# ooowedyn/InkLayer

Measured on AMD Instinct MI355X. Metric: sketches/sec end-to-end (GroundingDINO+SAM) at 1024x1024, higher is better.
Workload: dtype f16 (MFMA, f32 accumulate; f32 residual/norm/softmax; split-f16 = fp32-grade operands for patch-embed, neck, mask decoder); 1 GPU; full GroundingDINO Swin-T + SAM ViT-H pipeline, batch=8 per GPU, 1024x1024 synthetic sketches, 16 boxes/sketch, random-init weights; global_batch=8, parallelism=image-parallel x1

## Files before the change

### include/inklayer_hip.h

```cpp
#ifndef INKLAYER_HIP_H
#define INKLAYER_HIP_H

#include <stdint.h>

#ifdef __cplusplus
extern "C" {
#endif

#define INK_ABI_VERSION 8
int ink_abi_version(void);

typedef struct InkGemm {
  const void* A;
  const void* W;
  const float* bias;
  const float* col_scale;
  const float* residual;
  const int32_t* row_map;
  void* C;
  int32_t M, N, K;
  int32_t lda, ldw, ldr, ldc;
  int32_t act;
  int32_t c_f16;
} InkGemm;
#define INK_ACT_NONE 0
#define INK_ACT_GELU 1
#define INK_ACT_RELU 2
int ink_gemm_f16(const InkGemm* p, void* stream);
int ink_gemm_set_variant(int32_t v);
int ink_gemm_query_variant(int32_t M, int32_t N, int32_t K);

int ink_layernorm_rows(const float* x, int64_t ldx, const float* gamma, const float* beta,
                       float eps, const int32_t* gather, int32_t rows_out, int32_t C,
                       void* out_f16, float* out_f32, int64_t ldo, int32_t act, int32_t split,
                       const float* add, int64_t ld_add, const int32_t* add_batch_rows, int32_t rows_per_batch,
                       void* stream);

int ink_add_cvt_f16(const float* a, const float* b, int64_t n_b, void* out_f16, int64_t n,
                    void* stream);
int ink_add_split_f16(const float* a, const float* b, int64_t n_b, void* out_f16, int64_t n, int32_t C,
                      void* stream);
int ink_add_f32(const float* a, const float* b, int64_t n_b, float* out, int64_t n, void* stream);

typedef struct InkAttn {
  const void* Q; const void* K; const void* V;
  void* O;
  int64_t ldq, ldk, ldv, ldo;
  int32_t n_batch, n_heads, n_q, n_k, head_dim;
  float scale;
  int32_t bias_mode;
  int32_t grid_w;
  const int32_t* q_batch_rows;
  const int32_t* kv_batch_rows;
  const float* rel_h; const float* rel_w;
  const void* rel_aug;
  const float* dense_bias; const float* dense_mask;
  int32_t n_mask; int32_t rel_f16;
  const int32_t* tok_rows;
  const void* pad_k; const void* pad_v;
} InkAttn;
int ink_flash_attn(const InkAttn* p, void* stream);

int ink_relpos_bias64_f16(const void* Q, int64_t ldq, const float* rel_pos_h, const float* rel_pos_w, int32_t n_batch,
                          int32_t n_heads, int32_t head_dim, float scale, void* out_h_f16, void* out_w_f16, void* stream);

int ink_relpos_bias(const void* Q, int64_t ldq, const float* rel_pos_h, const float* rel_pos_w,
                    int32_t S, int32_t n_batch, int32_t n_heads, int32_t head_dim, float scale,
                    const int32_t* tok_rows, float* out_h, float* out_w, void* out_aug_f16,
                    void* stream);

int ink_sam_patchify(const void* image_u8, int32_t h, int32_t w, int32_t L, int32_t P,
                     const float* mean3, const float* std3, int32_t chan_reverse, int32_t split,
                     void* out_f16, void* stream);

int ink_resize_bilinear_u8(const void* src_u8, int32_t h, int32_t w, void* dst_u8, int32_t oh, int32_t ow,
                           const int32_t* xbounds, const int32_t* xcoef, int32_t kx,
                           const int32_t* ybounds, const int32_t* ycoef, int32_t ky, void* tmp_u8,
                           void* stream);

int ink_im2col3x3_f16(const void* in_f16, int32_t B, int32_t H, int32_t W, int32_t C, void* out_f16,
                      void* stream);

int ink_sam_pe_encode(const float* coords01, const float* gauss, int32_t N, int32_t F,
                      const float* add, int32_t n_add, float* out, void* stream);

int ink_sam_prompt_tokens(const float* points, const int32_t* labels, int32_t n_pts, int32_t pad, const float* boxes,
                          const float* gauss, int32_t F, const float* point_emb, const float* not_a_point,
                          const float* out_tok, float input_size, int32_t P, float* out, void* stream);

int ink_sam_mask_embed(const float* mask, const float* emb, const int32_t* emb_rows, const float* params,
                       int32_t n_params, float eps, int32_t P, int32_t g, float* keys, void* split_f16, void* stream);

int ink_sam_mask_logits(const float* up, const float* hyper, int32_t n, int32_t g, int32_t C,
                        float* out, void* stream);

int ink_sam_postprocess(const float* low, int32_t n, int32_t S, int32_t L, int32_t in_h,
                        int32_t in_w, int32_t out_h, int32_t out_w, float thr, void* out_u8,
                        float* out_logits, void* stream);

int ink_ms_deform_attn_forward(const float* value, const int64_t* spatial_shapes_host,
                               const int64_t* level_start_index_host, const float* sampling_loc,
                               const float* attn_weight, int32_t B, int32_t S, int32_t M, int32_t C,
                               int32_t Q, int32_t L, int32_t P, int32_t im2col_step, float* out,
                               void* stream);

int ink_ms_deform_attn_forward_dev(const void* value, const int64_t* spatial_shapes,
                                   const int64_t* level_start_index, const void* sampling_loc,
                                   const void* attn_weight, int32_t dtype, int32_t B, int32_t S, int32_t M,
                                   int32_t C, int32_t Q, int32_t L, int32_t P, int32_t im2col_step,
                                   void* out, void* stream);
int ink_ms_deform_attn_backward_dev(const void* value, const int64_t* spatial_shapes,
                                    const int64_t* level_start_index, const void* sampling_loc,
                                    const void* attn_weight, const void* grad_output, int32_t dtype,
                                    int32_t B, int32_t S, int32_t M, int32_t C, int32_t Q, int32_t L,
                                    int32_t P, int32_t im2col_step, void* grad_value,
                                    void* grad_sampling_loc, void* grad_attn_weight, void* stream);

int ink_msda_fused(const void* value_f16, const float* proj, int64_t ldp, const float* ref,
                   int32_t ref_dim, int64_t ref_q_stride, int64_t ref_b_stride,
                   const int32_t* shapes_host, int32_t B, int32_t S, int32_t Q, void* out_f16,
                   void* stream);

int ink_swin_patchify(const void* image_u8, int32_t h, int32_t w, const float* mean3,
                      const float* std3, void* out_f16, void* stream);

int ink_layernorm_merge4(const float* x, int64_t ldx, const float* gamma, const float* beta, float eps,
                         const int32_t* gather4, int32_t rows, int32_t C, void* out_f16, void* stream);

int ink_groupnorm_nhwc(const float* x, int32_t B, int32_t T, int32_t C, int32_t G, const float* gamma,
                       const float* beta, float eps, float* stats_ws, float* out,
                       int64_t out_batch_stride, void* stream);

int ink_gather_rows(const float* x, int64_t ldx, int64_t x_batch_rows, const int32_t* idx,
                    int64_t idx_batch_stride, int32_t rows_per_batch, int32_t B, int32_t C,
                    void* out_f16, float* out_f32, void* stream);

int ink_biattn_fusion(const void* QV_f16, const void* KL_f16, int32_t B, int32_t S, int32_t T, int32_t E,
                      float scale, float* scores_ws, float* stats_ws, float* partial_ws, int32_t chunk,
                      void* out_v_f16, void* out_l_f16, void* stream);

int ink_attn_fewkeys(const void* Q, int64_t ldq, const void* K, int64_t ldk, const void* V, int64_t ldv,
                     int32_t B, int32_t n_q, int32_t n_k, int32_t n_heads, int32_t head_dim, float scale,
                     const uint8_t* blocked, const int32_t* q_batch_rows, const float* q_add, int32_t io_f32, void* O,
                     int64_t ldo, void* stream);

int ink_attn_fewq(const void* Q, int64_t ldq, const void* K, int64_t ldk, const void* V, int64_t ldv,
                  int32_t n_batch, int32_t n_q, int32_t n_k, int32_t n_heads, int32_t head_dim, float scale,
                  const int32_t* q_batch_rows, const int32_t* kv_batch_rows, const float* k_add, void* O, int64_t ldo,
                  void* stream);

int ink_biattn_colstats(const float* scores, int32_t B, int32_t S, int32_t HT, float* part_ws, float* stats, void* stream);

int ink_fusion_fold_workspace(int32_t B, int32_t S, int64_t* out_floats);
int ink_fusion_fold(float* v_f32, int32_t B, int32_t S, const float* lnv_g, const float* lnv_b, float eps,
                    const float* text_k_f32, const float* text_vl_f32, int64_t ld_text, int32_t T, const void* Wq_f16,
                    const float* bq, const void* Wvv_f16, const float* bvv, const void* Wo_f16, const float* bo,
                    const float* gamma_v, float scale, float* ws, void* out_l_f16, const float* pos, void* out16_pos,
                    void* out16, void* stream);

int ink_sam_upscale_pack(const void* ws_f16, void* blob_f16, void* stream);
int ink_sam_upscale_tail(const float* u0, int64_t ld_tok, int32_t n, int32_t g, const float* ln_g, const float* ln_b, float eps,
                         const void* blob_f16, const float* b3, const float* hyper, int32_t n_masks, float* low,
                         void* stream);

int ink_proj256_ln_pack(const void* ws_f16, void* blob_f16, void* stream);
int ink_proj256_ln(const float* a_f32, const void* blob_f16, const float* bias, const float* res_f32,
                   const int32_t* res_batch_rows, int32_t rows_per_batch, const float* ln_g, const float* ln_b, float eps,
                   int64_t rows, float* out_f32, void* out_split_f16, void* stream);

int ink_ffn256_pack_bytes(int32_t hid, int32_t with_pre, int64_t* out_bytes);
int ink_ffn256_pack(const void* w1_f16, const float* b1, const void* w2_f16, int32_t hid, const void* wpre_f16, void* blob,
                    void* stream);
int ink_ffn256_fused(const void* x_f16, int64_t ldx, const float* res_f32, const void* blob, const float* b2,
                     const float* ln_g, const float* ln_b, float eps, int32_t M, int32_t hid, const float* pre_bias,
                     const float* pre_ln_g, const float* pre_ln_b, float* out_f32, void* stream);

int ink_topk_rowmax(const float* logits, int32_t B, int32_t S, int32_t T, int32_t K, int32_t* out_idx,
                    float* out_val, void* cand_ws, void* stream);

int ink_sine_embed4(const float* ref, const float* dim_t, int32_t N, void* out_f16, void* stream);

int ink_box_refine(const float* delta, int64_t ldd, const float* ref, int32_t N, int32_t ref_is_logit,
                   float* out, void* stream);
// ... 157 lines not shown
```

### inklayer_amd/_lib.py

```python
from __future__ import annotations

import ctypes as C
import os
from pathlib import Path

_LIB_PATH = Path(__file__).resolve().parent / "lib" / "libinklayer_hip.so"
_lib = None

c_void_p, c_int, c_i64, c_float = C.c_void_p, C.c_int32, C.c_int64, C.c_float


class InkGemm(C.Structure):
    _fields_ = [
        ("A", c_void_p), ("W", c_void_p), ("bias", c_void_p), ("col_scale", c_void_p),
        ("residual", c_void_p), ("row_map", c_void_p), ("C", c_void_p),
        ("M", c_int), ("N", c_int), ("K", c_int),
        ("lda", c_int), ("ldw", c_int), ("ldr", c_int), ("ldc", c_int),
        ("act", c_int), ("c_f16", c_int),
    ]


class InkAttn(C.Structure):
    _fields_ = [
        ("Q", c_void_p), ("K", c_void_p), ("V", c_void_p), ("O", c_void_p),
        ("ldq", c_i64), ("ldk", c_i64), ("ldv", c_i64), ("ldo", c_i64),
        ("n_batch", c_int), ("n_heads", c_int), ("n_q", c_int), ("n_k", c_int),
        ("head_dim", c_int), ("scale", c_float), ("bias_mode", c_int), ("grid_w", c_int),
        ("q_batch_rows", c_void_p), ("kv_batch_rows", c_void_p),
        ("rel_h", c_void_p), ("rel_w", c_void_p), ("rel_aug", c_void_p),
        ("dense_bias", c_void_p), ("dense_mask", c_void_p), ("n_mask", c_int), ("rel_f16", c_int),
        ("tok_rows", c_void_p), ("pad_k", c_void_p), ("pad_v", c_void_p),
    ]


SIGNATURES = {
    "ink_abi_version": [],
    "ink_gemm_f16": [C.POINTER(InkGemm), c_void_p],
    "ink_gemm_set_variant": [c_int],
    "ink_gemm_query_variant": [c_int, c_int, c_int],
    "ink_layernorm_rows": [c_void_p, c_i64, c_void_p, c_void_p, c_float, c_void_p, c_int, c_int,
                           c_void_p, c_void_p, c_i64, c_int, c_int, c_void_p, c_i64, c_void_p, c_int, c_void_p],
    "ink_add_split_f16": [c_void_p, c_void_p, c_i64, c_void_p, c_i64, c_int, c_void_p],
    "ink_add_cvt_f16": [c_void_p, c_void_p, c_i64, c_void_p, c_i64, c_void_p],
    "ink_add_f32": [c_void_p, c_void_p, c_i64, c_void_p, c_i64, c_void_p],
    "ink_flash_attn": [C.POINTER(InkAttn), c_void_p],
    "ink_sam_patchify": [c_void_p, c_int, c_int, c_int, c_int, C.POINTER(c_float), C.POINTER(c_float),
                         c_int, c_int, c_void_p, c_void_p],
    "ink_im2col3x3_f16": [c_void_p, c_int, c_int, c_int, c_int, c_void_p, c_void_p],
    "ink_resize_bilinear_u8": [c_void_p, c_int, c_int, c_void_p, c_int, c_int, c_void_p, c_void_p, c_int,
                               c_void_p, c_void_p, c_int, c_void_p, c_void_p],
    "ink_sam_pe_encode": [c_void_p, c_void_p, c_int, c_int, c_void_p, c_int, c_void_p, c_void_p],
    "ink_sam_mask_logits": [c_void_p, c_void_p, c_int, c_int, c_int, c_void_p, c_void_p],
    "ink_sam_prompt_tokens": [c_void_p, c_void_p, c_int, c_int, c_void_p, c_void_p, c_int, c_void_p, c_void_p,
                              c_void_p, c_float, c_int, c_void_p, c_void_p],
    "ink_sam_mask_embed": [c_void_p, c_void_p, c_void_p, c_void_p, c_int, c_float, c_int, c_int, c_void_p, c_void_p,
                           c_void_p],
    "ink_sam_postprocess": [c_void_p, c_int, c_int, c_int, c_int, c_int, c_int, c_int, c_float,
                            c_void_p, c_void_p, c_void_p],
    "ink_sam_amg_stats": [c_void_p, c_int, c_void_p, c_int, c_void_p, c_int, c_int, c_int, c_int, c_int, c_int, C.c_double,
                          C.c_double, c_int, c_int, c_int, c_int, c_void_p, c_void_p, c_void_p, c_void_p],
    "ink_mask_rle_counts": [c_void_p, c_void_p, c_int, c_int, c_int, c_void_p, c_void_p],
    "ink_mask_rle_write": [c_void_p, c_void_p, c_int, c_int, c_int, c_void_p, c_void_p, c_void_p],
    "ink_mask_small_regions_workspace_ints": [c_int, c_int, c_int, C.POINTER(c_i64)],
    "ink_mask_small_regions": [c_void_p, c_int, c_int, c_int, c_int, c_int, c_void_p, c_void_p, c_void_p, c_void_p,
                               c_void_p],
    "ink_box_nms": [c_void_p, c_void_p, c_int, c_float, c_void_p, c_void_p, c_void_p, c_void_p],
    "ink_ms_deform_attn_forward": [c_void_p, C.POINTER(c_i64), C.POINTER(c_i64), c_void_p, c_void_p, c_int,
                                   c_int, c_int, c_int, c_int, c_int, c_int, c_int, c_void_p, c_void_p],
    "ink_ms_deform_attn_forward_dev": [c_void_p, c_void_p, c_void_p, c_void_p, c_void_p, c_int, c_int, c_int, c_int,
                                       c_int, c_int, c_int, c_int, c_int, c_void_p, c_void_p],
    "ink_ms_deform_attn_backward_dev": [c_void_p, c_void_p, c_void_p, c_void_p, c_void_p, c_void_p, c_int, c_int, c_int,
                                        c_int, c_int, c_int, c_int, c_int, c_int, c_void_p, c_void_p, c_void_p,
                                        c_void_p],
    "ink_msda_fused": [c_void_p, c_void_p, c_i64, c_void_p, c_int, c_i64, c_i64, C.POINTER(c_int), c_int,
                       c_int, c_int, c_void_p, c_void_p],
    "ink_swin_patchify": [c_void_p, c_int, c_int, C.POINTER(c_float), C.POINTER(c_float), c_void_p, c_void_p],
    "ink_layernorm_merge4": [c_void_p, c_i64, c_void_p, c_void_p, c_float, c_void_p, c_int, c_int, c_void_p,
                             c_void_p],
    "ink_groupnorm_nhwc": [c_void_p, c_int, c_int, c_int, c_int, c_void_p, c_void_p, c_float, c_void_p,
                           c_void_p, c_i64, c_void_p],
    "ink_gather_rows": [c_void_p, c_i64, c_i64, c_void_p, c_i64, c_int, c_int, c_int, c_void_p, c_void_p,
                        c_void_p],
    "ink_biattn_fusion": [c_void_p, c_void_p, c_int, c_int, c_int, c_int, c_float, c_void_p, c_void_p,
                          c_void_p, c_int, c_void_p, c_void_p, c_void_p],
    "ink_biattn_colstats": [c_void_p, c_int, c_int, c_int, c_void_p, c_void_p, c_void_p],
    "ink_fusion_fold_workspace": [c_int, c_int, C.POINTER(c_i64)],
    "ink_relpos_bias64_f16": [c_void_p, c_i64, c_void_p, c_void_p, c_int, c_int, c_int, c_float, c_void_p, c_void_p, c_void_p],
    "ink_proj256_ln_pack": [c_void_p, c_void_p, c_void_p],
    "ink_proj256_ln": [c_void_p, c_void_p, c_void_p, c_void_p, c_void_p, c_int, c_void_p, c_void_p, c_float, c_i64, c_void_p,
                       c_void_p, c_void_p],
    "ink_sam_upscale_pack": [c_void_p, c_void_p, c_void_p],
    "ink_sam_upscale_tail": [c_void_p, c_i64, c_int, c_int, c_void_p, c_void_p, c_float, c_void_p, c_void_p, c_void_p,
                             c_int, c_void_p, c_void_p],
    "ink_ffn256_pack_bytes": [c_int, c_int, C.POINTER(c_i64)],
    "ink_ffn256_pack": [c_void_p, c_void_p, c_void_p, c_int, c_void_p, c_void_p, c_void_p],
    "ink_ffn256_fused": [c_void_p, c_i64, c_void_p, c_void_p, c_void_p, c_void_p, c_void_p, c_float, c_int, c_int,
                         c_void_p, c_void_p, c_void_p, c_void_p, c_void_p],
    "ink_fusion_fold": [c_void_p, c_int, c_int, c_void_p, c_void_p, c_float, c_void_p, c_void_p, c_i64, c_int, c_void_p,
                        c_void_p, c_void_p, c_void_p, c_void_p, c_void_p, c_void_p, c_float, c_void_p, c_void_p, c_void_p,
                        c_void_p, c_void_p, c_void_p],
    "ink_attn_fewkeys": [c_void_p, c_i64, c_void_p, c_i64, c_void_p, c_i64, c_int, c_int, c_int, c_int, c_int,
                         c_float, c_void_p, c_void_p, c_void_p, c_int, c_void_p, c_i64, c_void_p],
    "ink_attn_fewq": [c_void_p, c_i64, c_void_p, c_i64, c_void_p, c_i64, c_int, c_int, c_int, c_int, c_int,
                      c_float, c_void_p, c_void_p, c_void_p, c_void_p, c_i64, c_void_p],
    "ink_topk_rowmax": [c_void_p, c_int, c_int, c_int, c_int, c_void_p, c_void_p, c_void_p, c_void_p],
    "ink_sine_embed4": [c_void_p, c_void_p, c_int, c_void_p, c_void_p],
    "ink_box_refine": [c_void_p, c_i64, c_void_p, c_int, c_int, c_void_p, c_void_p],
    "ink_mask_cleanup_workspace_ints": [c_int, c_int, c_int, c_int, C.POINTER(c_i64)],
    "ink_mask_cleanup": [c_void_p, c_int, c_int, c_int, c_int, c_int, C.c_double, c_void_p, c_void_p, c_void_p,
                         c_void_p, c_void_p],
    "ink_mask_sketch_iou_counts": [c_void_p, c_void_p, c_int, c_int, c_int, c_void_p, c_void_p, c_void_p],
    "ink_refine_sketch_planes": [c_void_p, c_int, c_int, c_void_p, c_void_p, c_void_p],
    "ink_bitplane_pack": [c_void_p, c_int, c_int, c_int, c_int, c_void_p, c_void_p],
    "ink_refine_depth_samples": [c_void_p, c_int, c_void_p, c_void_p, c_int, c_int, c_int, c_void_p, c_void_p, c_void_p],
    "ink_refine_pair_tables": [c_void_p, c_void_p, c_int, c_int, c_int, c_void_p, c_void_p, c_void_p, c_void_p,
                               c_void_p, c_void_p],
    "ink_refine_composite": [c_void_p, c_void_p, c_int, c_int, c_int, c_void_p, c_void_p, c_void_p],
    "ink_refine_relabel_clean": [c_void_p, c_void_p, c_int, c_int, c_void_p, c_void_p],
    "ink_refine_grow_workspace": [c_int, c_int, C.POINTER(c_i64), C.POINTER(c_i64)],
    "ink_refine_grow": [c_void_p, c_void_p, c_int, c_int, c_void_p, c_void_p, c_void_p, c_void_p, c_void_p, c_void_p,
                        c_int, c_void_p, c_void_p],
    "ink_refine_query_dists": [c_void_p, c_void_p, c_void_p, c_int, c_int, c_int, c_void_p, c_void_p],
    "ink_refine_finalize": [c_void_p, c_void_p, c_int, c_void_p, c_int, c_int, c_void_p, c_void_p, c_void_p, c_void_p],
    "ink_host_sparse_sample": [c_void_p, c_int, c_int, c_void_p, c_int, c_void_p],
    "ink_host_assign_unlabeled": [c_void_p, c_int, c_void_p, c_int, c_void_p, c_void_p, c_void_p, c_int, c_void_p],
    "ink_depth_patchify": [c_void_p, c_int, c_int, c_int, c_int, c_int, c_int, C.POINTER(C.c_double), C.POINTER(C.c_double),
                           c_int, c_void_p, c_void_p],
    "ink_resize_bilinear_ac_nhwc": [c_void_p, c_int, c_int, c_int, c_int, c_int, c_int, c_void_p, c_void_p, c_void_p],
    "ink_im2col3x3_ex_f16": [c_void_p, c_int, c_int, c_int, c_int, c_int, c_int, c_void_p, c_void_p],
    "ink_conv3x3_f16": [c_void_p, c_int, c_int, c_int, c_int, c_void_p, c_int, c_void_p, c_int, c_int, c_int, c_void_p,
                        c_void_p, c_int, c_void_p],
    "ink_layers_otsu_planes": [c_void_p, c_int, c_int, c_int, c_int, c_void_p, c_void_p, c_void_p, c_void_p],
    "ink_layers_dilate": [c_void_p, c_int, c_int, c_int, c_int, c_int, c_void_p, c_void_p, c_void_p],
    "ink_layers_border_band": [c_void_p, c_int, c_int, c_int, c_int, c_void_p, c_void_p],
    "ink_layers_components_workspace_ints": [c_int, c_int, c_int, C.POINTER(c_i64)],
    "ink_layers_components": [c_void_p, c_int, c_int, c_int, c_int, c_void_p, c_void_p, c_void_p, c_void_p],
    "ink_layers_chamfer_workspace_ints": [c_int, c_int, c_int, C.POINTER(c_i64)],
    "ink_layers_chamfer": [c_void_p, c_void_p, c_int, c_int, c_int, c_int, c_int, c_void_p, c_void_p, c_void_p, c_void_p,
                           c_void_p, c_void_p],
    "ink_layers_mask_tables": [c_void_p, c_int, c_int, c_int, c_void_p, c_void_p, c_void_p],
    "ink_layers_assemble": [c_void_p, c_void_p, c_void_p, c_void_p, c_void_p, c_int, c_int, c_int, c_void_p, c_void_p,
                            c_void_p, c_void_p],
    "ink_layers_composite": [c_void_p, c_void_p, c_int, c_int, c_void_p, c_void_p],
    "ink_layers_gray": [c_void_p, c_int, c_int, c_int, c_void_p, c_void_p],
    "ink_layers_rgba": [c_void_p, c_void_p, c_int, c_int, c_int, c_void_p, c_void_p],
    "ink_inp_contrast": [c_void_p, c_int, c_int, c_float, c_void_p, c_void_p, c_void_p],
    "ink_inp_bilateral": [c_void_p, c_int, c_int, c_void_p, c_void_p, c_void_p],
    "ink_inp_mask_prepare": [c_void_p, c_int, c_int, c_int, c_int, c_void_p, c_void_p, c_void_p],
    "ink_inp_resize_u8": [c_void_p, c_int, c_int, c_int, c_void_p, c_int, c_int, c_void_p, c_void_p, c_int,
                          c_void_p, c_void_p, c_int, c_void_p, c_void_p],
    "ink_inp_condition": [c_void_p, c_void_p, c_int, c_int, c_void_p, c_void_p],
    "ink_inp_cleanup": [c_void_p, c_int, c_int, c_void_p, c_void_p, c_void_p, c_void_p, c_void_p],
    "ink_inp_soft_blend": [c_void_p, c_void_p, c_void_p, c_int, c_int, c_void_p, c_void_p, c_void_p, c_void_p],
    "ink_inp_luma": [c_void_p, c_int, c_int, c_int, c_void_p, c_void_p],
    "ink_inp_unsharp": [c_void_p, c_int, c_int, c_int, C.c_uint32, C.c_uint32, c_int, c_int, c_void_p, c_void_p, c_void_p],
    "ink_inp_rgba_cut": [c_void_p, c_void_p, c_int, c_int, c_void_p, c_void_p],
    "ink_vis_gray_min": [c_void_p, c_int, c_int, c_int, c_void_p, c_void_p],
    "ink_vis_colour": [c_void_p, c_int, c_void_p, c_int, c_int, c_void_p, c_void_p, c_int, c_int, c_void_p, c_void_p],
    "ink_eval_label_ranks": [c_void_p, c_int, c_int, c_int, c_void_p, c_void_p, c_int, c_void_p, c_void_p, c_void_p],
    "ink_eval_contingency": [c_void_p, c_int, c_int, c_void_p, c_int, c_void_p, c_int, c_int, c_int, c_int, c_void_p,
                             c_void_p],
    "ink_eval_label_boxes": [c_void_p, c_int, c_int, c_int, c_void_p, c_void_p],
    "ink_eval_paint_labels": [c_void_p, c_void_p, c_int, c_int, c_int, c_void_p, c_void_p],
    "ink_relpos_bias": [c_void_p, c_i64, c_void_p, c_void_p, c_int, c_int, c_int, c_int, c_float,
                        c_void_p, c_void_p, c_void_p, c_void_p, c_void_p],
}


class InkLayerHipError(RuntimeError):
    pass


def lib_path() -> Path:
    return Path(os.environ.get("INKLAYER_HIP_LIB", _LIB_PATH))


def lib() -> C.CDLL:
    global _lib
    if _lib is None:
        p = lib_path()
        if not p.exists():
            raise InkLayerHipError(
                f"{p} not found: build it with `python -m inklayer_amd.build` "
                "(there is no CPU/eager fallback for the InkLayer hot path)")
        try:
            import torch
        except ImportError:
            pass
        l = C.CDLL(str(p))
        for name, argtypes in SIGNATURES.items():
# ... 11 lines not shown
```

### inklayer_amd/csrc/gemm.hip

```cpp
#include <stdlib.h>

#include "common.h"
#include "../../include/inklayer_hip.h"

namespace {

template <int BK> struct Swz;
template <> struct Swz<64> {
  static __device__ __forceinline__ int f(int row) { return row & 7; }
};
template <> struct Swz<32> {
  static __device__ __forceinline__ int f(int row) { return (-(row >> 2)) & 3; }
};

typedef __attribute__((address_space(1))) const void* gptr_t;
typedef __attribute__((address_space(3))) void* lptr_t;

__device__ __forceinline__ bool residual_preloaded(const InkGemm& p) {
  return p.residual && p.act == INK_ACT_NONE && !p.col_scale;
}

template <int TM>
__device__ __forceinline__ void wave_rows(int (&rows)[TM], const InkGemm& p, int mw, int lane) {
#pragma unroll
  for (int ti = 0; ti < TM; ++ti) {
    const int m = mw + ti * 16 + (lane & 15);
    int r = -1;
    if (m < p.M) r = p.row_map ? p.row_map[m] : m;
    rows[ti] = r;
  }
}

template <int TM, int TN>
__device__ __forceinline__ void init_wave_tile(f32x4 (&acc)[TM][TN], const InkGemm& p, const int (&rows)[TM], int nw,
                                               int lane) {
  const int fq = lane >> 4;
  const bool pre = residual_preloaded(p);
#pragma unroll
  for (int ti = 0; ti < TM; ++ti) {
    const int r = pre ? rows[ti] : -1;
    const float* rp = p.residual + (size_t)max(r, 0) * p.ldr + nw + fq * 4;
#pragma unroll
    for (int j = 0; j < TN; ++j) {
      acc[ti][j] = (f32x4){0.f, 0.f, 0.f, 0.f};
      if (r >= 0 && nw + j * 16 + fq * 4 < p.N) acc[ti][j] = *(const f32x4*)(rp + j * 16);
    }
  }
}

template <int TM, int TN>
__device__ __forceinline__ void add_bias_wave_tile(f32x4 (&acc)[TM][TN], const InkGemm& p, int nw, int lane) {
  const int fq = lane >> 4;
#pragma unroll
  for (int j = 0; j < TN; ++j) {
    const int n = nw + j * 16 + fq * 4;
    f32x4 bv = (f32x4){0.f, 0.f, 0.f, 0.f};
    if (p.bias && n < p.N) bv = *(const f32x4*)(p.bias + n);
#pragma unroll
    for (int ti = 0; ti < TM; ++ti) acc[ti][j] += bv;
  }
}

template <int TM, int TN, int OUT, int MODE = -1>
__device__ __forceinline__ void store_wave_tile(f32x4 (&acc)[TM][TN], const InkGemm& p, char* er,
                                                const int (&rows)[TM], int nw, int lane) {
  constexpr bool F16O = OUT == 1;
  constexpr int WNC = TN * 16, EP = WNC * 4 + 16;
  constexpr int ES = OUT == 0 ? 4 : 8;
  constexpr int CPRW = WNC / ES;
  constexpr int NIT = (16 * CPRW + 63) / 64;
  const int fr = lane & 15, fq = lane >> 4;
  const bool wide16 = OUT != 0 && (p.ldc % 8 == 0);
  const bool res_late = MODE < 0 && p.residual && !residual_preloaded(p);
  const int act = MODE < 0 ? p.act : MODE;
  const bool scaled = MODE < 0 && p.col_scale != nullptr;
  int row_of[NIT], n_of[NIT];
#pragma unroll
  for (int it = 0; it < NIT; ++it) {
    const int c = it * 64 + lane;
    row_of[it] = c < 16 * CPRW ? c / CPRW : 16;
    n_of[it] = nw + (c % CPRW) * ES;
  }

  add_bias_wave_tile<TM, TN>(acc, p, nw, lane);

#pragma unroll
  for (int ti = 0; ti < TM; ++ti) {
#pragma unroll
    for (int j = 0; j < TN; ++j) {
      f32x4 v = acc[ti][j];
      if (act == INK_ACT_GELU) {
#pragma unroll
        for (int r = 0; r < 4; ++r) v[r] = gelu_erf(v[r]);
      } else if (act == INK_ACT_RELU) {
#pragma unroll
        for (int r = 0; r < 4; ++r) v[r] = fmaxf(v[r], 0.f);
      }
      if (scaled) {
        const int n = nw + j * 16 + fq * 4;
        if (n < p.N) v *= *(const f32x4*)(p.col_scale + n);
      }
      if (F16O) {
        *(f16x4*)(er + fr * EP + (j * 16 + fq * 4) * 2) = (f16x4){(f16)v[0], (f16)v[1], (f16)v[2], (f16)v[3]};
      } else {
        *(f32x4*)(er + fr * EP + (j * 16 + fq * 4) * 4) = v;
      }
    }
#pragma unroll
    for (int it = 0; it < NIT; ++it) {
      int r = __builtin_amdgcn_ds_bpermute((row_of[it] & 15) << 2, rows[ti]);
      if (row_of[it] >= 16 || n_of[it] >= p.N) r = -1;
      if (r >= 0) {
        const int c_n = n_of[it];
        const char* src = er + row_of[it] * EP + (c_n - nw) * (F16O ? 2 : 4);
        if (F16O) {
          f16x8 d = *(const f16x8*)src;
          f16* dst = (f16*)p.C + (size_t)r * p.ldc + c_n;
          if (res_late) {
            const float* rp = p.residual + (size_t)r * p.ldr + c_n;
#pragma unroll
            for (int e = 0; e < 8; ++e)
              if (c_n + e < p.N) d[e] = (f16)((float)d[e] + rp[e]);
          }
          if (wide16 && c_n + 8 <= p.N) {
            *(f16x8*)dst = d;
          } else {
            *(f16x4*)dst = (f16x4){d[0], d[1], d[2], d[3]};
            if (c_n + 8 <= p.N) *(f16x4*)(dst + 4) = (f16x4){d[4], d[5], d[6], d[7]};
          }
        } else {
          f32x4 d = *(const f32x4*)src;
          if (res_late) d += *(const f32x4*)(p.residual + (size_t)r * p.ldr + c_n);
          *(f32x4*)((float*)p.C + (size_t)r * p.ldc + c_n) = d;
        }
      }
    }
  }
}

__device__ __forceinline__ void tile_of(int id, int ntm, int ntn, int group_m, int& mt, int& nt) {
  if (group_m > 1) {
    const int per = group_m * ntn;
    const int first = (id / per) * group_m;
    const int gsz = min(ntm - first, group_m);
    mt = first + (id % per) % gsz;
    nt = (id % per) / gsz;
  } else {
    mt = id / ntn;
    nt = id % ntn;
  }
}

constexpr int NS = 2;
// ... 118 lines not shown
  constexpr int TM = 8, WNC = 16 * TN;
  constexpr int AHEAD = RING - 2;
  constexpr int AG = 4;
  constexpr int EP = WNC * 4 + 16;
  static_assert(8 * 16 * EP <= RING * GRAN, "patch fits");
  extern __shared__ __attribute__((aligned(16))) char smem[];
  const int tid = threadIdx.x, lane = tid & 63;
  const int wave = __builtin_amdgcn_readfirstlane(tid >> 6);
  const int grp = wave >> 2, wn = wave & 3;
  const int fr = lane & 15, fq = lane >> 4;

  const int ntn = (p.N + BN - 1) / BN, ntm = (p.M + BM - 1) / BM;
  int mt, nt;
  tile_of(xcd_remap(blockIdx.x, ntm * ntn), ntm, ntn, group_m, mt, nt);
  const int m0 = mt * BM, n0 = nt * BN;
  const int G = p.K / BK;
  const f16* __restrict__ A = (const f16*)p.A;
  const f16* __restrict__ W = (const f16*)p.W;
  const f16* srcA[IT_A];
  const f16* srcW[IT_W + (W_TAIL ? 1 : 0)];
#pragma unroll
  for (int it = 0; it < IT_A; ++it) {
    const int pch = it * NT + tid, row = pch / CPR, lch = (pch % CPR) ^ Swz<BK>::f(row);
    srcA[it] = A + (size_t)min(m0 + row, p.M - 1) * p.lda + lch * 8;
  }
#pragma unroll
  for (int it = 0; it < IT_W + (W_TAIL ? 1 : 0); ++it) {
    const int pch = it * NT + tid, row = min(pch / CPR, BN - 1), lch = (pch % CPR) ^ Swz<BK>::f(row);
    srcW[it] = W + (size_t)min(n0 + row, p.N - 1) * p.ldw + lch * 8;
  }
  auto dma = [&](int g, int slot) {
    char* base = smem + slot * GRAN;
#pragma unroll
    for (int it = 0; it < IT_A; ++it)
      __builtin_amdgcn_global_load_lds((gptr_t)(srcA[it] + g * BK), (lptr_t)(base + (it * NT + wave * 64) * 16), 16, 0, 0);
#pragma unroll
    for (int it = 0; it < IT_W; ++it)
      __builtin_amdgcn_global_load_lds((gptr_t)(srcW[it] + g * BK), (lptr_t)(base + TILE_A + (it * NT + wave * 64) * 16), 16, 0, 0);
    if (W_TAIL && grp == 0)
      __builtin_amdgcn_global_load_lds((gptr_t)(srcW[IT_W] + g * BK), (lptr_t)(base + TILE_A + (IT_W * NT + wave * 64) * 16), 16, 0, 0);
  };
  auto wait_ahead = [&]() {
    if (W_TAIL && grp == 0) {
      asm volatile("s_waitcnt vmcnt(%0)" ::"n"((AHEAD - 1) * (LOADS + 1)) : "memory");
    } else {
      asm volatile("s_waitcnt vmcnt(%0)" ::"n"((AHEAD - 1) * LOADS) : "memory");
    }
  };
  auto slot_end = [&]() {
    __builtin_amdgcn_sched_barrier(0);
    __builtin_amdgcn_s_barrier();
    __builtin_amdgcn_sched_barrier(0);
  };

  int rows[TM];
  wave_rows<TM>(rows, p, m0 + grp * 128, lane);
#pragma unroll
  for (int g = 0; g < AHEAD; ++g) dma(g, g);
  f32x4 acc[TM][TN];
  init_wave_tile<TM, TN>(acc, p, rows, n0 + wn * WNC, lane);
  if (residual_preloaded(p)) {
    asm volatile("s_waitcnt vmcnt(0)" ::: "memory");
  } else {
    wait_ahead();
  }
  slot_end();
  if (grp == 1) slot_end();

  const int offA = (grp * 128 + fr) * ROWB;
  const int offW = (wn * WNC + fr) * ROWB;
  const int co = (fq ^ Swz<BK>::f(fr)) << 4;
  f16x8 a[AG], w[TN];
  int cslot = 0, islot = AHEAD % RING;
  auto iter = [&](int g) __attribute__((always_inline)) {
    const char* bA = smem + cslot * GRAN;
    const char* bW = bA + TILE_A;
#pragma unroll
    for (int i = 0; i < AG; ++i) a[i] = *(const f16x8*)(bA + offA + i * 16 * ROWB + co);
#pragma unroll
    for (int j = 0; j < TN; ++j) w[j] = *(const f16x8*)(bW + offW + j * 16 * ROWB + co);
    if (g + AHEAD < G) {
      dma(g + AHEAD, islot);
      wait_ahead();
    } else {
      asm volatile("s_waitcnt vmcnt(0)" ::: "memory");
    }
    slot_end();
    asm volatile("s_waitcnt lgkmcnt(0)" ::: "memory");
    __builtin_amdgcn_sched_barrier(0);
    __builtin_amdgcn_s_setprio(1);
#pragma unroll
    for (int i0 = 0; i0 < TM; i0 += AG) {
#pragma unroll
      for (int i = 0; i < AG; ++i) {
#pragma unroll
        for (int j = 0; j < TN; ++j)
          acc[i0 + i][j] = __builtin_amdgcn_mfma_f32_16x16x32_f16(w[j], a[i], acc[i0 + i][j], 0, 0, 0);
        if (i0 + AG < TM) {
          a[i] = *(const f16x8*)(bA + offA + (i0 + AG + i) * 16 * ROWB + co);
          __builtin_amdgcn_sched_barrier(0);
        }
      }
    }
    __builtin_amdgcn_s_setprio(0);
    slot_end();
    cslot = (cslot + 1 == RING) ? 0 : cslot + 1;
    islot = (islot + 1 == RING) ? 0 : islot + 1;
  };
  for (int g = 0; g < G; ++g) iter(g);
  if (grp == 0) slot_end();

  char* er = smem + wave * (16 * EP);
  const bool plain = !p.col_scale && !(p.residual && !residual_preloaded(p));
  if (p.c_f16) {
    if (plain && p.act == INK_ACT_GELU) {
      store_wave_tile<TM, TN, 1, INK_ACT_GELU>(acc, p, er, rows, n0 + wn * WNC, lane);
    } else if (plain && p.act == INK_ACT_NONE) {
      store_wave_tile<TM, TN, 1, INK_ACT_NONE>(acc, p, er, rows, n0 + wn * WNC, lane);
    } else {
      store_wave_tile<TM, TN, 1>(acc, p, er, rows, n0 + wn * WNC, lane);
    }
  } else {
    if (plain && p.act == INK_ACT_NONE) {
      store_wave_tile<TM, TN, 0, INK_ACT_NONE>(acc, p, er, rows, n0 + wn * WNC, lane);
    } else {
      store_wave_tile<TM, TN, 0>(acc, p, er, rows, n0 + wn * WNC, lane);
    }
  }
}

static int launch_gemm_pp(const InkGemm& p, hipStream_t s, int group_m) {
  if (p.K / 32 < PP_RING) return INK_ERR_ARG;
  constexpr int BN = 64 * PP_TN;
  constexpr int lds = PP_RING * (256 + BN) * 32 * 2;
  static_assert(lds <= 160 * 1024, "LDS budget");
  static bool attr = ((void)hipFuncSetAttribute((const void*)gemm_f16_nt_pp,
                                                hipFuncAttributeMaxDynamicSharedMemorySize, lds), true);
  (void)attr;
  const int ntiles = ((p.M + 255) / 256) * ((p.N + BN - 1) / BN);
  hipLaunchKernelGGL(gemm_f16_nt_pp, dim3(ntiles), dim3(512), lds, s, p, group_m);
  return ink_launch_status();
}

template <int BM, int BN, int BK, int WM, int WN>
static int launch_gemm(const InkGemm& p, hipStream_t s, int group_m = 1) {
  constexpr int lds = NS * (BM + BN) * BK * 2;
  static_assert(lds <= 160 * 1024, "LDS budget");
  static bool attr = ((void)hipFuncSetAttribute((const void*)gemm_f16_nt<BM, BN, BK, WM, WN>,
                                                hipFuncAttributeMaxDynamicSharedMemorySize, lds), true);
  (void)attr;
  const int ntm = (p.M + BM - 1) / BM, ntn = (p.N + BN - 1) / BN;
  hipLaunchKernelGGL((gemm_f16_nt<BM, BN, BK, WM, WN>), dim3(ntm * ntn), dim3(WM * WN * 64), lds, s, p, group_m);
  return ink_launch_status();
}

struct ConvGeom {
  int H, W, C, OH, OW, stride;
};
__device__ __attribute__((aligned(128))) const uint32_t g_conv_zero_row[32] = {};

template <int BK, bool RELU_IN>
__global__ __launch_bounds__(256) void conv3x3_f16_nt(InkGemm p, ConvGeom g) {
  constexpr int BM = 128, BN = 128, WM = 2, WN = 2;
  constexpr int NT = WM * WN * 64;
  constexpr int CPR = BK / 8;
  constexpr int ROWB = BK * 2;
  constexpr int TILE_A = BM * ROWB, TILE_W = BN * ROWB;
  constexpr int STAGE = TILE_A + TILE_W;
  constexpr int IT_A = (BM * CPR) / NT, IT_W = (BN * CPR) / NT;
  constexpr int TM = BM / WM / 16, TN = BN / WN / 16;
  extern __shared__ __attribute__((aligned(16))) char smem[];

  const int tid = threadIdx.x;
  const int lane = tid & 63;
  const int wave = tid >> 6;
  const int wm = wave / WN, wn = wave % WN;

  const int ntn = (p.N + BN - 1) / BN;
  const int ntm = (p.M + BM - 1) / BM;
  int mt, nt;
  tile_of(xcd_remap(blockIdx.x, ntm * ntn), ntm, ntn, 1, mt, nt);
  const int m0 = mt * BM;
  const int n0 = nt * BN;

  const f16* __restrict__ A = (const f16*)p.A;
  const f16* __restrict__ W = (const f16*)p.W;

  const f16* ctrA[IT_A];
  const f16* zeroA[IT_A];
  int maskA[IT_A];
  const f16* srcW[IT_W];
#pragma unroll
  for (int it = 0; it < IT_A; ++it) {
    const int pch = it * NT + tid;
    const int row = pch / CPR;
    const int lch = (pch % CPR) ^ Swz<BK>::f(row);
    const int m = min(m0 + row, p.M - 1);
    const int b = m / (g.OH * g.OW);
    const int rem = m - b * (g.OH * g.OW);
    const int oy = rem / g.OW;
    const int iy = oy * g.stride, ix = (rem - oy * g.OW) * g.stride;
    ctrA[it] = A + (((size_t)b * g.H + iy) * g.W + ix) * g.C + lch * 8;
    zeroA[it] = (const f16*)g_conv_zero_row + lch * 8;
    const int rowok = (iy > 0 ? 1 : 0) | 2 | (iy + 1 < g.H ? 4 : 0);
    const int colok = (ix > 0 ? 1 : 0) | 2 | (ix + 1 < g.W ? 4 : 0);
    int mask = 0;
#pragma unroll
    for (int ky = 0; ky < 3; ++ky)
      if ((rowok >> ky) & 1) mask |= colok << (ky * 3);
    maskA[it] = mask;
  }
#pragma unroll
  for (int it = 0; it < IT_W; ++it) {
    const int pch = it * NT + tid;
    const int row = pch / CPR;
    const int lch = (pch % CPR) ^ Swz<BK>::f(row);
    srcW[it] = W + (size_t)min(n0 + row, p.N - 1) * p.ldw + lch * 8;
  }

  int s_tap = 0, s_c0 = 0;
  auto stage = [&](int buf, int kt) {
    char* base = smem + buf * STAGE;
    const int ky = s_tap / 3, kx = s_tap - ky * 3;
    const ptrdiff_t doff = ((ptrdiff_t)(ky - 1) * g.W + (kx - 1)) * g.C + s_c0;
#pragma unroll
    for (int it = 0; it < IT_A; ++it) {
      const f16* src = ((maskA[it] >> s_tap) & 1) ? ctrA[it] + doff : zeroA[it];
      __builtin_amdgcn_global_load_lds((gptr_t)src, (lptr_t)(base + (it * NT + wave * 64) * 16), 16, 0, 0);
    }
#pragma unroll
    for (int it = 0; it < IT_W; ++it)
      __builtin_amdgcn_global_load_lds((gptr_t)(srcW[it] + kt * BK), (lptr_t)(base + TILE_A + (it * NT + wave * 64) * 16), 16, 0, 0);
    s_c0 += BK;
    if (s_c0 == g.C) {
      s_c0 = 0;
      ++s_tap;
    }
  };

  int rows[TM];
  wave_rows<TM>(rows, p, m0 + wm * (BM / WM), lane);
  f32x4 acc[TM][TN];

  const int fr = lane & 15, fq = lane >> 4;
  const int offA = (wm * (BM / WM) + fr) * ROWB;
  const int offW = (wn * (BN / WN) + fr) * ROWB;
  const int swz = Swz<BK>::f(fr);

  const int nk = p.K / BK;
  auto compute = [&](int cur) {
    const char* bA = smem + cur * STAGE;
    const char* bW = bA + TILE_A;
#pragma unroll
    for (int kk = 0; kk < BK / 32; ++kk) {
      f16x8 a[TM], w[TN];
      const int co = ((kk * 4 + fq) ^ swz) << 4;
#pragma unroll
      for (int j = 0; j < TN; ++j) w[j] = *(const f16x8*)(bW + offW + j * 16 * ROWB + co);
#pragma unroll
      for (int i = 0; i < TM; ++i) {
        a[i] = *(const f16x8*)(bA + offA + i * 16 * ROWB + co);
        if (RELU_IN) a[i] = __builtin_elementwise_max(a[i], (f16x8)(f16)0);
      }
#pragma unroll
      for (int i = 0; i < TM; ++i)
#pragma unroll
        for (int j = 0; j < TN; ++j)
          acc[i][j] = __builtin_amdgcn_mfma_f32_16x16x32_f16(w[j], a[i], acc[i][j], 0, 0, 0);
    }
  };

  stage(0, 0);
  init_wave_tile<TM, TN>(acc, p, rows, n0 + wn * (BN / WN), lane);
  for (int kt = 0; kt < nk; ++kt) {
    asm volatile("s_waitcnt vmcnt(0)" ::: "memory");
    __syncthreads();
    if (kt + 1 < nk) stage((kt + 1) & 1, kt + 1);
    compute(kt & 1);
  }

  constexpr int WNC = BN / WN;
  constexpr int EP = WNC * 4 + 16;
  static_assert(WM * WN * 16 * EP <= NS * STAGE, "epilogue patch must fit in the staging LDS");
  __syncthreads();
  char* er = smem + wave * (16 * EP);
  if (p.c_f16 == 1) {
    store_wave_tile<TM, TN, 1>(acc, p, er, rows, n0 + wn * WNC, lane);
  } else {
    store_wave_tile<TM, TN, 0>(acc, p, er, rows, n0 + wn * WNC, lane);
  }
}

template <int BK, bool RELU_IN>
static int launch_conv3x3(const InkGemm& p, const ConvGeom& g, hipStream_t s) {
  constexpr int lds = NS * (128 + 128) * BK * 2;
  static bool attr = ((void)hipFuncSetAttribute((const void*)conv3x3_f16_nt<BK, RELU_IN>,
                                                hipFuncAttributeMaxDynamicSharedMemorySize, lds), true);
  (void)attr;
  const int ntm = (p.M + 127) / 128, ntn = (p.N + 127) / 128;
  hipLaunchKernelGGL((conv3x3_f16_nt<BK, RELU_IN>), dim3(ntm * ntn), dim3(256), lds, s, p, g);
  return ink_launch_status();
}

}

extern "C" int ink_conv3x3_f16(const void* in_f16, int32_t B, int32_t H, int32_t W, int32_t C, const void* wt_f16,
                               int32_t N, const float* bias, int32_t stride, int32_t relu_in, int32_t act,
                               const float* residual, void* out, int32_t out_f16, void* stream) {
  INK_CHECK_ARG(in_f16 && wt_f16 && out);
  INK_CHECK_ARG(B > 0 && H > 0 && W > 0 && C > 0 && N > 0);
  INK_CHECK_ARG(C % 32 == 0 && N % 4 == 0);
  INK_CHECK_ARG(stride == 1 || stride == 2);
  INK_CHECK_ARG(((uintptr_t)in_f16 & 15) == 0 && ((uintptr_t)wt_f16 & 15) == 0);
  INK_CHECK_ARG(((uintptr_t)out & 15) == 0 && ((uintptr_t)residual & 15) == 0 && ((uintptr_t)bias & 15) == 0);
  INK_CHECK_ARG(relu_in == 0 || relu_in == 1);
  INK_CHECK_ARG(act == INK_ACT_NONE || act == INK_ACT_RELU);
  INK_CHECK_ARG(out_f16 == 0 || out_f16 == 1);
  const int OH = (H - 1) / stride + 1, OW = (W - 1) / stride + 1;
  const int64_t M = (int64_t)B * OH * OW;
  INK_CHECK_ARG(M <= INT32_MAX - 128 && (int64_t)9 * C <= INT32_MAX);
  InkGemm p = {};
  p.A = in_f16;
  p.W = wt_f16;
  p.bias = bias;
  p.residual = residual;
  p.C = out;
  p.M = (int32_t)M;
  p.N = N;
  p.K = 9 * C;
  p.lda = p.ldw = 9 * C;
  p.ldr = p.ldc = N;
  p.act = act;
  p.c_f16 = out_f16;
  const ConvGeom g = {H, W, C, OH, OW, stride};
  hipStream_t s = (hipStream_t)stream;
  if (C % 64 == 0) return relu_in ? launch_conv3x3<64, true>(p, g, s) : launch_conv3x3<64, false>(p, g, s);
  return relu_in ? launch_conv3x3<32, true>(p, g, s) : launch_conv3x3<32, false>(p, g, s);
}

static int g_variant = -1;
extern "C" int ink_gemm_query_variant(int32_t M, int32_t N, int32_t K) {
  if (K % 64 != 0) return 32;
  if (N % 320 == 0 && K >= 128 && (long)((M + 255) / 256) * (N / 320) >= 384) return 45;
  const long tiles256 = (long)((M + 255) / 256) * ((N + 255) / 256);
  const bool n_fits = (N % 256 == 0) || N >= 1024;
  return (tiles256 >= 200 && n_fits) ? 10 : 0;
}
extern "C" int ink_abi_version(void) { return INK_ABI_VERSION; }
extern "C" int ink_gemm_set_variant(int32_t v) {
  INK_CHECK_ARG(v == -1 || v == 0 || v == 10 || v == 45);
  g_variant = v;
  return INK_OK;
}

extern "C" int ink_gemm_f16(const InkGemm* pp, void* stream) {
  INK_CHECK_ARG(pp != nullptr);
  const InkGemm& p = *pp;
  INK_CHECK_ARG(p.A && p.W && p.C);
  INK_CHECK_ARG(p.M > 0 && p.N > 0 && p.K > 0);
  INK_CHECK_ARG(p.K % 32 == 0 && p.N % 4 == 0);
  INK_CHECK_ARG(p.lda % 8 == 0 && p.ldw % 8 == 0 && p.lda >= p.K && p.ldw >= p.K);
  INK_CHECK_ARG(p.ldc % 4 == 0 && p.ldc >= p.N);
  INK_CHECK_ARG(!p.residual || (p.ldr % 4 == 0 && p.ldr >= p.N));
  INK_CHECK_ARG(((uintptr_t)p.A & 15) == 0 && ((uintptr_t)p.W & 15) == 0);
  INK_CHECK_ARG(((uintptr_t)p.C & 15) == 0);
  INK_CHECK_ARG(p.act >= 0 && p.act <= 2);
  INK_CHECK_ARG(p.c_f16 == 0 || p.c_f16 == 1);
  hipStream_t s = (hipStream_t)stream;
  if (p.K % 64 != 0) return launch_gemm<128, 128, 32, 2, 2>(p, s);
  int v = g_variant;
  if (v < 0) v = ink_gemm_query_variant(p.M, p.N, p.K);
  switch (v) {
    case 10: return launch_gemm<256, 256, 64, 4, 4>(p, s, 4);
    case 45: return launch_gemm_pp(p, s, 4);
    default: return launch_gemm<128, 128, 64, 2, 2>(p, s);
  }
}
```

Before: 120.3 sketches/s.

## Add warp-specialized streaming GEMM for tall skinny N=192 K=192 projections

Adds a new GEMM kernel for large-M, small-N, small-K shapes. A fifth producer wave DMAs A row-blocks into LDS, up to three buffers deep, while four compute waves keep a whole resident N-slice of W in LDS and stream across many M steps. Each block walks a run of M steps so W is loaded once per block. The kernel also has a fused bias/activation/scale/residual epilogue staged through LDS patches. Dispatch sends N==192, K==192, M>=65536 to this path, which targets the Swin-T stage-1 linear layers where the 256x256 tiles waste work. The gain depends on the hand-written vmcnt waits being correct, and the dispatch now ignores the K%64 fallback for this variant.

```diff
diff --git a/include/inklayer_hip.h b/include/inklayer_hip.h
--- a/include/inklayer_hip.h
+++ b/include/inklayer_hip.h
@@ -29,6 +29,7 @@
 int ink_gemm_f16(const InkGemm* p, void* stream);
 int ink_gemm_set_variant(int32_t v);
 int ink_gemm_query_variant(int32_t M, int32_t N, int32_t K);
+int ink_gemm_stream_f16(const InkGemm* p, void* stream);
 
 int ink_layernorm_rows(const float* x, int64_t ldx, const float* gamma, const float* beta,
                        float eps, const int32_t* gather, int32_t rows_out, int32_t C,
diff --git a/inklayer_amd/_lib.py b/inklayer_amd/_lib.py
--- a/inklayer_amd/_lib.py
+++ b/inklayer_amd/_lib.py
@@ -36,6 +36,7 @@
 SIGNATURES = {
     "ink_abi_version": [],
     "ink_gemm_f16": [C.POINTER(InkGemm), c_void_p],
+    "ink_gemm_stream_f16": [C.POINTER(InkGemm), c_void_p],
     "ink_gemm_set_variant": [c_int],
     "ink_gemm_query_variant": [c_int, c_int, c_int],
     "ink_layernorm_rows": [c_void_p, c_i64, c_void_p, c_void_p, c_float, c_void_p, c_int, c_int,
diff --git a/inklayer_amd/csrc/gemm.hip b/inklayer_amd/csrc/gemm.hip
--- a/inklayer_amd/csrc/gemm.hip
+++ b/inklayer_amd/csrc/gemm.hip
@@ -1,4 +1,6 @@
 #include <stdlib.h>
+
+#include <algorithm>
 
 #include "common.h"
 #include "../../include/inklayer_hip.h"
@@ -423,6 +425,250 @@
   const int ntm = (p.M + BM - 1) / BM, ntn = (p.N + BN - 1) / BN;
   hipLaunchKernelGGL((gemm_f16_nt<BM, BN, BK, WM, WN>), dim3(ntm * ntn), dim3(WM * WN * 64), lds, s, p, group_m);
   return ink_launch_status();
+}
+
+constexpr int ST_G = 3;
+constexpr int ST_SPW = 8;
+
+template <int OUT>
+struct StreamPatch {
+  static constexpr int EP = ST_G * 16 * (OUT == 0 ? 4 : 2) + 16;
+};
+constexpr int ST_PATCH = 4 * 16 * StreamPatch<0>::EP;
+
+template <int TN, int OUT, int MODE>
+__device__ __forceinline__ void stream_store_tile(f32x4 (&acc)[1][TN], const InkGemm& p, char* er, int orow, int nw,
+                                                  int lane) {
+  constexpr bool F16O = OUT == 1;
+  constexpr int EP = StreamPatch<OUT>::EP;
+  constexpr int ES = OUT == 0 ? 4 : 8;
+  constexpr int CPRW = ST_G * 16 / ES;
+  constexpr int NIT = (16 * CPRW + 63) / 64;
+  const int fr = lane & 15, fq = lane >> 4;
+  const bool wide16 = OUT != 0 && (p.ldc % 8 == 0);
+  const bool res_late = MODE < 0 && p.residual && !residual_preloaded(p);
+  const int act = MODE < 0 ? p.act : MODE;
+  const bool scaled = MODE < 0 && p.col_scale != nullptr;
+#pragma unroll
+  for (int g0 = 0; g0 < TN; g0 += ST_G) {
+    const int gw = nw + g0 * 16;
+#pragma unroll
+    for (int j = 0; j < ST_G; ++j) {
+      f32x4 v = acc[0][g0 + j];
+      if (act == INK_ACT_GELU) {
+#pragma unroll
+        for (int r = 0; r < 4; ++r) v[r] = gelu_erf(v[r]);
+      } else if (act == INK_ACT_RELU) {
+#pragma unroll
+        for (int r = 0; r < 4; ++r) v[r] = fmaxf(v[r], 0.f);
+      }
+      if (scaled) {
+        const int n = gw + j * 16 + fq * 4;
+        if (n < p.N) v *= *(const f32x4*)(p.col_scale + n);
+      }
+      if (F16O) {
+        *(f16x4*)(er + fr * EP + (j * 16 + fq * 4) * 2) = (f16x4){(f16)v[0], (f16)v[1], (f16)v[2], (f16)v[3]};
+      } else {
+        *(f32x4*)(er + fr * EP + (j * 16 + fq * 4) * 4) = v;
+      }
+    }
+#pragma unroll
+    for (int it = 0; it < NIT; ++it) {
+      const int c = it * 64 + lane;
+      const int prow = c < 16 * CPRW ? c / CPRW : 16;
+      const int c_n = gw + (c % CPRW) * ES;
+      int r = __builtin_amdgcn_ds_bpermute((prow & 15) << 2, orow);
+      if (prow >= 16 || c_n >= p.N) r = -1;
+      if (r >= 0) {
+        const char* src = er + prow * EP + (c_n - gw) * (F16O ? 2 : 4);
+        if (F16O) {
+          f16x8 d = *(const f16x8*)src;
+          f16* dst = (f16*)p.C + (size_t)r * p.ldc + c_n;
+          if (res_late) {
+            const float* rp = p.residual + (size_t)r * p.ldr + c_n;
+#pragma unroll
+            for (int e = 0; e < 8; ++e)
+              if (c_n + e < p.N) d[e] = (f16)((float)d[e] + rp[e]);
+          }
+          if (wide16 && c_n + 8 <= p.N) {
+            *(f16x8*)dst = d;
+          } else {
+            *(f16x4*)dst = (f16x4){d[0], d[1], d[2], d[3]};
+            if (c_n + 8 <= p.N) *(f16x4*)(dst + 4) = (f16x4){d[4], d[5], d[6], d[7]};
+          }
+        } else {
+          f32x4 d = *(const f32x4*)src;
+          if (res_late) d += *(const f32x4*)(p.residual + (size_t)r * p.ldr + c_n);
+          *(f32x4*)((float*)p.C + (size_t)r * p.ldc + c_n) = d;
+        }
+      }
+    }
+  }
+}
+
+template <int MUL>
+__device__ __forceinline__ void wait_vmcnt_steps(int n) {
+#define INK_W(N) case N: asm volatile("s_waitcnt vmcnt(%0)" ::"n"(N * MUL) : "memory"); break;
+  switch (n) {
+    INK_W(1) INK_W(2) INK_W(3) INK_W(4) INK_W(5) INK_W(6) INK_W(7) INK_W(8) INK_W(9) INK_W(10) INK_W(11) INK_W(12)
+    default: asm volatile("s_waitcnt vmcnt(0)" ::: "memory");
+  }
+#undef INK_W
+}
+
+template <int WM, int WN, int TN>
+__global__ __launch_bounds__(320) __attribute__((amdgpu_waves_per_eu(3))) void gemm_f16_nt_stream(InkGemm p, int spw, int nb) {
+  static_assert(WM * WN == 4 && TN % ST_G == 0, "4 compute waves, whole epilogue groups");
+  constexpr int BM = 16 * WM, SN = 16 * TN * WN;
+  extern __shared__ __attribute__((aligned(16))) char smem[];
+  const int tid = threadIdx.x, lane = tid & 63;
+  const int wave = __builtin_amdgcn_readfirstlane(tid >> 6);
+  const int cpr = p.K >> 3, rowb = p.K * 2, ks = p.K >> 5;
+  const int lg = (cpr & 15) == 0 ? 4 : (cpr & 7) == 0 ? 3 : 2;
+  auto swz = [&](int row) { return (row >> (4 - lg)) & ((1 << lg) - 1); };
+
+  const int nsl = (p.N + SN - 1) / SN;
+  const int nsteps = (p.M + BM - 1) / BM;
+  const int id = xcd_remap(blockIdx.x, gridDim.x);
+  const int n0 = (id % nsl) * SN;
+  const int s0 = (id / nsl) * spw, s1 = min(s0 + spw, nsteps);
+  if (s0 >= s1) return;
+  char* sW = smem;
+  char* sA = smem + SN * rowb;
+  const int abuf = BM * rowb;
+
+  if (wave == 4) {
+    const f16* __restrict__ A = (const f16*)p.A;
+    const f16* __restrict__ W = (const f16*)p.W;
+    auto dma_rows = [&](const f16* base, int ld, int row0, int rmax, int nrows, char* dst) {
+      const int npieces = (nrows * cpr) >> 6;
+      const int dq = 64 / cpr, dr = 64 % cpr;
+      int row = lane / cpr, pc = lane % cpr;
+      for (int q = 0; q < npieces; ++q) {
+        const f16* src = base + (size_t)min(row0 + row, rmax) * ld + ((pc ^ swz(row)) << 3);
+        __builtin_amdgcn_global_load_lds((gptr_t)src, (lptr_t)(dst + q * 1024), 16, 0, 0);
+        row += dq;
+        pc += dr;
+        if (pc >= cpr) {
+          pc -= cpr;
+          ++row;
+        }
+      }
+    };
+    const int ahead = nb - 1;
+    dma_rows(W, p.ldw, n0, p.N - 1, SN, sW);
+    for (int d = 0; d < ahead; ++d)
+      if (s0 + d < s1) dma_rows(A, p.lda, (s0 + d) * BM, p.M - 1, BM, sA + d * abuf);
+    int slot = ahead % nb;
+    for (int s = s0; s < s1; ++s) {
+      if (ahead == 2 && s + 1 < s1) {
+        wait_vmcnt_steps<WM>(ks);
+      } else {
+        asm volatile("s_waitcnt vmcnt(0)" ::: "memory");
+      }
+      __builtin_amdgcn_s_barrier();
+      if (s + ahead < s1) dma_rows(A, p.lda, (s + ahead) * BM, p.M - 1, BM, sA + slot * abuf);
+      slot = slot + 1 == nb ? 0 : slot + 1;
+    }
+    return;
+  }
+
+  const int wm = wave / WN, wn = wave % WN;
+  const int fr = lane & 15, fq = lane >> 4;
+  const int nw = n0 + wn * (TN * 16);
+  char* er = sA + nb * abuf + wave * (16 * StreamPatch<0>::EP);
+  char* sB = sA + nb * abuf + ST_PATCH + wave * (TN * 64);
+  if (lane < TN * 4) {
+    const int n = nw + lane * 4;
+    f32x4 b = (f32x4){0.f, 0.f, 0.f, 0.f};
+    if (p.bias && n < p.N) b = *(const f32x4*)(p.bias + n);
+    *(f32x4*)(sB + lane * 16) = b;
+  }
+  int rows[1];
+  const bool plain = !p.col_scale && !(p.residual && !residual_preloaded(p));
+  const int offA = (wm * 16 + fr) * rowb, offW = (wn * (TN * 16) + fr) * rowb;
+  const int sw = swz(fr);
+  int slot = 0;
+
+  for (int s = s0; s < s1; ++s) {
+    f32x4 acc[1][TN];
+    wave_rows<1>(rows, p, s * BM + wm * 16, lane);
+    init_wave_tile<1, TN>(acc, p, rows, nw, lane);
+    __builtin_amdgcn_sched_barrier(0);
+    __builtin_amdgcn_s_barrier();
+    __builtin_amdgcn_sched_barrier(0);
+    asm volatile("" ::: "memory");
+
+    const char* bA = sA + slot * abuf + offA;
+    const char* bW = sW + offW;
+    for (int kk = 0; kk < ks; ++kk) {
+      const int co = ((kk * 4 + fq) ^ sw) << 4;
+      const f16x8 a = *(const f16x8*)(bA + co);
+#pragma unroll
+      for (int j = 0; j < TN; ++j) {
+        const f16x8 w = *(const f16x8*)(bW + j * 16 * rowb + co);
+        acc[0][j] = __builtin_amdgcn_mfma_f32_16x16x32_f16(w, a, acc[0][j], 0, 0, 0);
+      }
+    }
+    slot = slot + 1 == nb ? 0 : slot + 1;
+
+#pragma unroll
+    for (int j = 0; j < TN; ++j) acc[0][j] += *(const f32x4*)(sB + (j * 16 + fq * 4) * 4);
+    if (p.c_f16) {
+      if (plain && p.act == INK_ACT_GELU) {
+        stream_store_tile<TN, 1, INK_ACT_GELU>(acc, p, er, rows[0], nw, lane);
+      } else if (plain && p.act == INK_ACT_NONE) {
+        stream_store_tile<TN, 1, INK_ACT_NONE>(acc, p, er, rows[0], nw, lane);
+      } else if (plain) {
+        stream_store_tile<TN, 1, INK_ACT_RELU>(acc, p, er, rows[0], nw, lane);
+      } else {
+        stream_store_tile<TN, 1, -1>(acc, p, er, rows[0], nw, lane);
+      }
+    } else {
+      if (plain && p.act == INK_ACT_GELU) {
+        stream_store_tile<TN, 0, INK_ACT_GELU>(acc, p, er, rows[0], nw, lane);
+      } else if (plain && p.act == INK_ACT_NONE) {
+        stream_store_tile<TN, 0, INK_ACT_NONE>(acc, p, er, rows[0], nw, lane);
+      } else if (plain) {
+        stream_store_tile<TN, 0, INK_ACT_RELU>(acc, p, er, rows[0], nw, lane);
+      } else {
+        stream_store_tile<TN, 0, -1>(acc, p, er, rows[0], nw, lane);
+      }
+    }
+  }
+}
+
+constexpr int ST_KMAX = 384;
+template <int WM, int WN, int TN>
+static constexpr int stream_lds(int K, int nb) {
+  return (16 * TN * WN + nb * 16 * WM) * K * 2 + ST_PATCH + 4 * TN * 64;
+}
+constexpr int ST_LDS_2WG = 80 * 1024;
+
+template <int WM, int WN, int TN>
+static int launch_gemm_stream(const InkGemm& p, hipStream_t s) {
+  static_assert(stream_lds<WM, WN, TN>(WM == 2 ? ST_KMAX : 32, 2) <= 160 * 1024, "LDS budget");
+  static bool attr = ((void)hipFuncSetAttribute((const void*)gemm_f16_nt_stream<WM, WN, TN>,
+                                                hipFuncAttributeMaxDynamicSharedMemorySize, 160 * 1024), true);
+  (void)attr;
+  const int nb = stream_lds<WM, WN, TN>(p.K, 3) <= ST_LDS_2WG ? 3 : 2;
+  const int lds = stream_lds<WM, WN, TN>(p.K, nb);
+  if (lds > 160 * 1024) return INK_ERR_ARG;
+  const int nsl = (p.N + 16 * TN * WN - 1) / (16 * TN * WN);
+  const int nsteps = (p.M + 16 * WM - 1) / (16 * WM);
+  const int spw = std::max(1, std::min(ST_SPW * (WM == 2 ? 2 : 1), (nsteps + 3) / 4));
+  const int nrg = (nsteps + spw - 1) / spw;
+  hipLaunchKernelGGL((gemm_f16_nt_stream<WM, WN, TN>), dim3(nsl * nrg), dim3(320), lds, s, p, spw, nb);
+  return ink_launch_status();
+}
+
+static int launch_gemm_stream_any(const InkGemm& p, hipStream_t s) {
+  if (p.K > ST_KMAX) return INK_ERR_ARG;
+  const int frags = (p.N + 15) / 16;
+  const bool wide = ((frags + 8) / 9) * 9 <= ((frags + 5) / 6) * 6;
+  if (wide && stream_lds<4, 1, 9>(p.K, 2) <= ST_LDS_2WG) return launch_gemm_stream<4, 1, 9>(p, s);
+  if (!wide && stream_lds<4, 1, 6>(p.K, 2) <= ST_LDS_2WG) return launch_gemm_stream<4, 1, 6>(p, s);
+  return launch_gemm_stream<2, 2, 3>(p, s);
 }
 
 struct ConvGeom {
@@ -611,6 +857,7 @@
 
 static int g_variant = -1;
 extern "C" int ink_gemm_query_variant(int32_t M, int32_t N, int32_t K) {
+  if (N == 192 && K == 192 && M >= 65536) return 60;
   if (K % 64 != 0) return 32;
   if (N % 320 == 0 && K >= 128 && (long)((M + 255) / 256) * (N / 320) >= 384) return 45;
   const long tiles256 = (long)((M + 255) / 256) * ((N + 255) / 256);
@@ -624,7 +871,7 @@
   return INK_OK;
 }
 
-extern "C" int ink_gemm_f16(const InkGemm* pp, void* stream) {
+static int gemm_f16_run(const InkGemm* pp, void* stream, int v) {
   INK_CHECK_ARG(pp != nullptr);
   const InkGemm& p = *pp;
   INK_CHECK_ARG(p.A && p.W && p.C);
@@ -638,12 +885,16 @@
   INK_CHECK_ARG(p.act >= 0 && p.act <= 2);
   INK_CHECK_ARG(p.c_f16 == 0 || p.c_f16 == 1);
   hipStream_t s = (hipStream_t)stream;
+  if (v < 0) v = ink_gemm_query_variant(p.M, p.N, p.K);
+  if (v == 60) return launch_gemm_stream_any(p, s);
   if (p.K % 64 != 0) return launch_gemm<128, 128, 32, 2, 2>(p, s);
-  int v = g_variant;
-  if (v < 0) v = ink_gemm_query_variant(p.M, p.N, p.K);
   switch (v) {
     case 10: return launch_gemm<256, 256, 64, 4, 4>(p, s, 4);
     case 45: return launch_gemm_pp(p, s, 4);
     default: return launch_gemm<128, 128, 64, 2, 2>(p, s);
   }
 }
+
+extern "C" int ink_gemm_f16(const InkGemm* pp, void* stream) { return gemm_f16_run(pp, stream, g_variant); }
+
+extern "C" int ink_gemm_stream_f16(const InkGemm* pp, void* stream) { return gemm_f16_run(pp, stream, 60); }
```

Measured after the change: 119.9 sketches/s. No clear change (-0.3%).
